# divideon/xvc

Hardware: AMD Instinct MI355X
Metric: hot-path frame passes/s (TZ + sub-pel ME, MC, transform + RDOQ + dequant + inverse, deblock, pad, PSNR parts), bit-exact vs the reference's classes (higher is better)
Workload: dtype u16; 1 GPU; 1920x1080 yuv420p 30fps synthetic, QP 32, internal bitdepth 10, 16x16 CUs, TZ range 96, RDOQ (RdoQuant::QuantRdo + CoeffSignHideRdo, picture-initial CABAC contexts); cus_per_picture=8160, parallelism=3 independent picture chains in flight

## Files before the change

### xvc_amd/csrc/k_quant.h

```cpp
#ifndef XVCGPU_K_QUANT_H_
#define XVCGPU_K_QUANT_H_

#include "dev_common.h"
#include "dev_tables.h"
#include "xvcgpu_internal.h"

struct TxBlockFlags {
  bool intra_pic;
  bool sign_hide;
  bool rdoq;
  int scan_order;
};
__device__ __forceinline__ TxBlockFlags tx_block_flags(int f) {
  return {(f & XVC_TXF_INTRA_PIC) != 0, !(f & XVC_TXF_NO_SIGN_HIDING), (f & XVC_TXF_RDOQ) != 0,
          (f >> XVC_TXF_SCAN_SHIFT) & 3};
}

__device__ __forceinline__ int rq_log2(int size) {
  return 31 - __clz(size);
}

struct BlockQuant {
  bool bias;
  int tshift;
  int scale;
  int shift;
  int size_bias_shift, size_bias_offset;
  int fq_shift;
  long long fq_offset;
  long long fast_offset;
  int iq_scale, iq_shift;
  int cost_scale;

  __device__ __forceinline__ int fwd(int a) const {
    return (int)(short)(int)((((long long)a * scale) + fq_offset) >> fq_shift);
  }
  __device__ __forceinline__ bool codes(int a) const { return fwd(a) != 0; }
  struct Fast {
    int16_t level, rem;
  };
  __device__ __forceinline__ Fast fast(int coeff) const {
    const int sign = coeff < 0 ? -1 : 1;
    const long long abs_coeff = d_abs(coeff);
    const int level = (int)(((abs_coeff * scale) + fast_offset) >> fq_shift);
    return {(int16_t)d_clip3(level * sign, -32768, 32767),
            (int16_t)(((abs_coeff * scale) - ((long long)level << fq_shift)) >> (fq_shift - 8))};
  }
  __device__ __forceinline__ int dequant(int level) const {
    const int prod = level * iq_scale;
    int cf;
    if (iq_shift > 0) cf = (prod + (1 << (iq_shift - 1))) >> iq_shift;
    else cf = (int)((unsigned)prod << -iq_shift);
    return (int)(short)d_clip3(cf, -32768, 32767);
  }
  __device__ __forceinline__ int err_of(int abs_coeff, int level) const {
    const long long orig_scaled =
        (((long long)abs_coeff * scale) + size_bias_offset) >> size_bias_shift;
    const long long quant_err = orig_scaled - ((long long)level << shift);
    return (int)(short)(quant_err >> (shift - 8));
  }
  __device__ __forceinline__ long long dist(int e) const {
    return ((long long)e * e) << cost_scale;
  }
  __device__ __forceinline__ long long zero_dist(int a) const {
    return ((long long)(a * a)) << cost_scale;
  }
};

__device__ __forceinline__ BlockQuant block_quant(int w, int h, int qp, int bd, bool intra_pic) {
  const int lsum = rq_log2(w) + rq_log2(h);
  int qpb = qp + 6 * (bd - 8);
  qpb = qpb > 0 ? qpb : 0;
  BlockQuant q;
  q.bias = (lsum & 1) != 0;
  q.tshift = 15 - bd - (lsum >> 1);
  q.scale = kFwdQuantScales[qpb % 6] * (q.bias ? 181 : 1);
  q.shift = 14 + qpb / 6 + q.tshift;
  q.size_bias_shift = q.bias ? 7 : 0;
  q.size_bias_offset = q.bias ? 64 : 0;
  q.fq_shift = q.shift + q.size_bias_shift;
  q.fq_offset = 1ll << (q.fq_shift - 1);
  q.fast_offset = (long long)((intra_pic ? 171ull : 85ull) << (q.fq_shift - 9));
  q.iq_scale = (kInvQuantScales[qpb % 6] << (qpb / 6)) * (q.bias ? 181 : 1);
  q.iq_shift = 6 - q.tshift + (q.bias ? 8 : 0);
  q.cost_scale = 15 - 2 * q.tshift - 2 * (bd - 8) + 2 * (q.bias ? 1 : 0);
  return q;
}
__device__ __forceinline__ BlockQuant block_quant(const xvcgpu_tx_block &b, int bd) {
  return block_quant(b.w, b.h, b.qp, bd, tx_block_flags(b.intra_pic).intra_pic);
}

struct TxStageShifts {
  int fwd1, fwd2, inv1, inv2;
  bool dct2_both;
};
__device__ __forceinline__ TxStageShifts tx_stage_shifts(int tx_hor, int tx_ver, int lgw, int lgh,
                                                         int bd) {
  const int hp_hor = tx_hor == XVC_TX_DCT2_LOW ? 0 : 2, hp_ver = tx_ver == XVC_TX_DCT2_LOW ? 0 : 2;
  auto dct2 = [](int t) { return t == XVC_TX_DEFAULT || t == XVC_TX_DCT2 || t == XVC_TX_DCT2_LOW; };
  return {lgw + bd - 9 + hp_hor, lgh + 6 + hp_ver, 7 + hp_ver, 20 - bd + hp_hor,
          dct2(tx_ver) && dct2(tx_hor)};
}
__device__ __forceinline__ TxStageShifts tx_stage_shifts_dst4(int bd) {
  TxStageShifts s = tx_stage_shifts(XVC_TX_DCT2_LOW, XVC_TX_DCT2_LOW, 2, 2, bd);
  s.dct2_both = false;
  return s;
}

__constant__ uint32_t kEntropyBits[128] = {
#include "entropy_bits.inc"
};
#define RQ_BYPASS 32768u
__device__ uint32_t gEntropyBits[128];

#define RQ_OFF(field) ((int)__builtin_offsetof(xvcgpu_rdoq_contexts, field))

__device__ __forceinline__ unsigned rq_bits(unsigned char state, int bin) {
  return kEntropyBits[state ^ bin];
}
__device__ __forceinline__ long long rq_bit_cost(unsigned bits, long long lambda) {
  return ((long long)bits * lambda) >> 16;
}

static_assert(sizeof(xvcgpu_rdoq_contexts) % 4 == 0, "whole words of contexts");
#define RQ_CTX_WORDS ((int)sizeof(xvcgpu_rdoq_contexts) / 4)
__device__ __forceinline__ void rq_stage_word(const uint32_t *table, uint32_t word, unsigned *cb8) {
#pragma unroll
  for (int k = 0; k < 4; k++) {
    const unsigned st8 = (word >> (8 * k)) & 127;
    *reinterpret_cast<uint2 *>(cb8 + 2 * k) = make_uint2(table[st8], table[st8 ^ 1]);
  }
}
__device__ __forceinline__ void rq_stage_costs(const uint32_t *table,
                                               const xvcgpu_rdoq_contexts *snap, unsigned *cb,
                                               int lane, int lanes) {
  const uint32_t *cw = reinterpret_cast<const uint32_t *>(snap);
  for (int wi = lane; wi < RQ_CTX_WORDS; wi += lanes) rq_stage_word(table, cw[wi], cb + 8 * wi);
}

__device__ __forceinline__ int rq_sig_ctx_base(bool luma, int posxy, int size_cls) {
  int start = posxy < 2 ? 6 : 0;
  start += luma && posxy < 5 ? 6 : 0;
  start += size_cls > 2 && luma ? 18 << (size_cls - 3 < 1 ? size_cls - 3 : 1) : 0;
  return 2 * ((luma ? RQ_OFF(sig_luma) : RQ_OFF(sig_chroma)) + start);
}
__device__ __forceinline__ int rq_greater1_off(bool luma) {
  return luma ? RQ_OFF(greater1_luma) : RQ_OFF(greater1_chroma);
}
__device__ __forceinline__ int rq_greater_start(bool luma, int posxy) {
  return luma ? (posxy < 3 ? 10 : (posxy < 10 ? 5 : 0)) : 0;
}
__device__ __forceinline__ int rq_greater_nn(int n, bool is_last) {
  return is_last ? 0 : (n < 4 ? n : 4) + 1;
}
__device__ __forceinline__ int rq_greater_ctx(bool luma, int posxy, int nn) {
  const int g1 = rq_greater1_off(luma);
  return nn == 0 ? 2 * g1 : 2 * (g1 + rq_greater_start(luma, posxy) + nn);
}

#endif
```

### xvc_amd/csrc/k_rdoq.h

```cpp
#ifndef XVCGPU_K_RDOQ_H_
#define XVCGPU_K_RDOQ_H_

#include "dev_common.h"
#include "k_me.h"
#include "k_me2.h"
#include "k_quant.h"
#include "k_rdoq4.h"
#include "k_rdoq_common.h"
#include "k_scan.h"
#include "xvcgpu_internal.h"


template <int G = 64, typename S, typename CF, typename LEV>
__device__ __forceinline__ int wave_rdoq(S &s, int lane, const BlockQuant &bq, int w, int h,
                                         bool luma, int scan_order, bool sign_hide,
                                         const xvcgpu_rdoq_contexts &ctx,
                                         const xvcgpu_rdoq_params &prm, CF cf, LEV lev,
                                         bool stage_ctx = true, bool clear_levels = true) {
  const int sbs = (w == 2 || h == 2) ? 1 : 2;
  const int sb_size = 1 << (2 * sbs);
  const int gw = w >> sbs, gh = h >> sbs;
  const int rw = w < 32 ? w : 32, rh = h < 32 ? h : 32;
  const int rgw = rw >> sbs, rgh = rh >> sbs;
  const int size_cls = (rq_log2(w) + rq_log2(h)) >> 1;
// ... 651 lines not shown
  l.part = base + 4 + 4 * (size_t)cap;
  return l;
}

__device__ __forceinline__ void rq_count_word(uint32_t v, int i, int end, int cnt[3]) {
#pragma unroll
  for (int k = 0; k < 4; k++) {
    const int c = (int)(signed char)(v >> (8 * k));
    const bool in = i + k < end;
    cnt[0] += in && c == 0;
    cnt[1] += in && c == 1;
    cnt[2] += in && c == 2;
  }
}
__device__ __forceinline__ int rq_wave_scan(int v) {
  const int lane = threadIdx.x & 63;
#pragma unroll
  for (int d = 1; d < 64; d <<= 1) {
    const int o = __shfl_up(v, d, 64);
    if (lane >= d) v += o;
  }
  return v;
}
template <int ROW>
__device__ __forceinline__ void rq_wave_totals_scan(int (&tot)[3][ROW]) {
  const int t = threadIdx.x;
  if (t < 64) {
#pragma unroll
    for (int k = 0; k < 3; k++) {
      int v = t < 16 ? tot[k][t] : 0;
#pragma unroll
      for (int d = 1; d < 16; d <<= 1) {
        const int o = __shfl_up(v, d, 64);
        if (t >= d) v += o;
      }
      if (t < 16) tot[k][16 + t] = v;
    }
  }
}
__device__ __forceinline__ void rq_scatter_word(uint32_t v, int i, int end, const RdoqLists &l,
                                                int pos[3]) {
#pragma unroll
  for (int k = 0; k < 4; k++) {
    const int c = (int)(signed char)(v >> (8 * k));
    if (i + k < end && c >= 0) l.list[c][pos[c]++] = i + k;
  }
}

__device__ __forceinline__ int rq_class_of(const xvcgpu_tx_block &b) {
  if (!rq4_takes(64, b.w, b.h, tx_block_flags(b.intra_pic).scan_order) || b.w > 32 || b.h > 32)
    return 2;
  const int n_sb = (b.w >> 2) * (b.h >> 2);
  return n_sb <= 4 ? 0 : (n_sb <= 16 ? 1 : 2);
}

__device__ __forceinline__ void rdoq_classify_kernel_body(int bd, const xvcgpu_tx_block *blocks, int n, const int16_t *coeffs, const uint32_t *d_off, int16_t *levels, int32_t *nnz_out, RdoqLists l) {
  const int bi = blockIdx.x * 4 + (int)(threadIdx.x >> 6);
  if (bi >= n) return;
  const int lane = threadIdx.x & 63;
  const xvcgpu_tx_block b = blocks[bi];
  const int w = b.w, h = b.h;
  const BlockQuant q = block_quant(b, bd);
  const int16_t *src = coeffs + d_off[bi];
  int16_t *dst = levels + d_off[bi];
  bool any = false;
  for (int i = lane; i < w * h; i += 64) any |= q.codes((short)d_abs((int)src[i]));
  if (__ballot(any)) {
    if (lane == 0) l.cls[bi] = (signed char)rq_class_of(b);
    return;
  }
  if (lane == 0) l.cls[bi] = -1;
  for (int i = lane; i < w * h; i += 64) dst[i] = 0;
  if (lane == 0 && nnz_out) nnz_out[bi] = 0;
}

__global__ void __launch_bounds__(256)
rdoq_classify_kernel(int bd, const xvcgpu_tx_block *blocks, int n, const int16_t *coeffs, const uint32_t *d_off, int16_t *levels, int32_t *nnz_out, RdoqLists l) {
  rdoq_classify_kernel_body(bd, blocks, n, coeffs, d_off, levels, nnz_out, l);
}

#define RQ_PROVE_BLOCKS 16
#define RQ_PROVE_MAX_CANDS 16

__device__ __forceinline__ int rq_prove_threshold(const BlockQuant &bq) {
  long long t = (long long)((double)bq.fq_offset / (double)bq.scale);
  while (t * bq.scale < bq.fq_offset) t++;
  while (t > 0 && (t - 1) * bq.scale >= bq.fq_offset) t--;
  return t > 32768 ? 32768 : (int)t;
}

template <class QAt>
__device__ __forceinline__ void rq_prove_candidate(const BlockQuant &bq, const xvcgpu_tx_block &b,
                                                   const xvcgpu_rdoq_params &prm,
                                                   const unsigned *cb, int x, int y, int a,
                                                   QAt qat, long long &gain, long long &gain_last,
                                                   long long &rhs, int &idx) {
  const int w = b.w, h = b.h, scan_order = tx_block_flags(b.intra_pic).scan_order;
  const bool luma = b.comp == 0;
  const long long lambda = prm.lambda;
  const int q = bq.fwd(a);
  int cnt, cnt1;
  {
    const int q0 = qat(x + 1, y), q1 = qat(x + 2, y), q2 = qat(x + 1, y + 1), q3 = qat(x, y + 1),
              q4 = qat(x, y + 2);
    cnt = (q0 > 0) + (q1 > 0) + (q2 > 0) + (q3 > 0) + (q4 > 0);
    cnt1 = (q0 > 1) + (q1 > 1) + (q2 > 1) + (q3 > 1) + (q4 > 1);
  }
  const int posxy = x + y;
  const int sig_base = rq_sig_ctx_base(luma, posxy, (rq_log2(w) + rq_log2(h)) >> 1);
  unsigned sig1 = 0xffffffffu;
  for (int nn = 0; nn <= cnt; nn++) {
    const unsigned v = cb[sig_base + 2 * nn + 1];
    sig1 = v < sig1 ? v : sig1;
  }
  const bool sub_dc = ((x | y) & 3) == 0 && (x | y) != 0;
  if (sub_dc) sig1 = 0;
  unsigned flag_min = RQ_BYPASS;
  auto meet = [&](int nn) {
    const int c = rq_greater_ctx(luma, posxy, nn);
    const unsigned v0 = cb[c], v1 = cb[c + 1];
    flag_min = v0 < flag_min ? v0 : flag_min;
    flag_min = v1 < flag_min ? v1 : flag_min;
  };
  meet(0);
  for (int n = 0; n <= cnt1; n++) meet(rq_greater_nn(n, false));
  const unsigned lvl_min = RQ_BYPASS + flag_min;
  long long d_best = bq.dist(a - bq.dequant(q));
  if (q > 1) {
    const long long d1 = bq.dist(a - bq.dequant(q - 1));
    d_best = d1 < d_best ? d1 : d_best;
  }
  const long long zd = bq.zero_dist(a);
  const long long coded = d_best + rq_bit_cost(sig1 + lvl_min, lambda);
  const long long coded_last = d_best + rq_bit_cost(lvl_min, lambda);
  gain = zd - (coded < zd ? coded : zd);
  gain_last = zd - coded_last;
  const unsigned lp = rq_last_pos_bits(cb, luma, w, h, scan_order, x, y);
  const int cbf_ctx = 2 * (!luma ? RQ_OFF(cbf_chroma)
                                 : ((prm.flags & XVC_RDOQ_INTRA_CU) ? RQ_OFF(cbf_luma)
                                                                    : RQ_OFF(root_cbf)));
  rhs = rq_bit_cost(cb[cbf_ctx + 1], lambda) - rq_bit_cost(cb[cbf_ctx], lambda) +
        rq_bit_cost(lp, lambda);
  constexpr unsigned long long inv0 = rq_pack_scan4_inv(0), inv1 = rq_pack_scan4_inv(1),
                               inv2 = rq_pack_scan4_inv(2);
  const unsigned long long inv = scan_order == 0 ? inv0 : (scan_order == 1 ? inv1 : inv2);
  const int kk = (int)((inv >> (4 * (((y & 3) << 2) | (x & 3)))) & 15ull);
  idx = (d_sb_scan_index(scan_order, w >> 2, h >> 2, x >> 2, y >> 2) << 4) + kk;
}

__global__ void __launch_bounds__(256)
rdoq_prove_zero_kernel(int bd, const xvcgpu_tx_block *blocks, int n, const int16_t *coeffs,
                       const uint32_t *d_off, int16_t *levels, int32_t *nnz_out,
                       const xvcgpu_rdoq_contexts *rq_ctx, const xvcgpu_rdoq_params *rq_prm,
                       RdoqLists l) {
  __shared__ __attribute__((aligned(16))) unsigned s_cb[2 * sizeof(xvcgpu_rdoq_contexts)];
  __shared__ unsigned short s_xy[16][RQ_PROVE_MAX_CANDS];
  __shared__ int s_idx[16][RQ_PROVE_MAX_CANDS];
  __shared__ long long s_gain[16][RQ_PROVE_MAX_CANDS];
  __shared__ int s_n[16];
  __shared__ int s_fail[16];
  __shared__ int s_ctx;
  const int g = threadIdx.x >> 4, gl = threadIdx.x & 15;
  const int base = blockIdx.x * RQ_PROVE_BLOCKS;
  if (threadIdx.x == 0) s_ctx = -1;
  __syncthreads();
  if ((int)threadIdx.x < RQ_PROVE_BLOCKS) {
    const int b2 = base + (int)threadIdx.x;
    if (b2 < n && l.cls[b2] >= 0) atomicMax(&s_ctx, (int)rq_prm[b2].ctx_index);
  }
  __syncthreads();
  const int wg_ctx = s_ctx;
  if (wg_ctx < 0) return;
  rq_stage_costs(gEntropyBits, &rq_ctx[wg_ctx], s_cb, (int)threadIdx.x, 256);
  __syncthreads();
  for (int sub = 0; sub < RQ_PROVE_BLOCKS / 16; sub++) {
    const int bi = base + sub * 16 + g;
    const bool live = bi < n && l.cls[bi < n ? bi : 0] >= 0;
    const xvcgpu_tx_block b = blocks[live ? bi : 0];
    const xvcgpu_rdoq_params prm = rq_prm[live ? bi : 0];
    if (gl == 0) {
      s_n[g] = 0;
      s_fail[g] = 0;
    }
    wave_sync();
    const BlockQuant bq = block_quant(b, bd);
    const int w = b.w, h = b.h;
    const int16_t *src = coeffs + d_off[live ? bi : 0];
    const bool tried = live && (int)prm.ctx_index == wg_ctx && w >= 4 && h >= 4 && w <= 32 &&
                       h <= 32 && (reinterpret_cast<uintptr_t>(src) & 7) == 0;
    auto qat = [&](int x, int y) {
      if (x >= w || y >= h) return 0;
      return bq.fwd((short)d_abs((int)src[y * w + x]));
    };
    if (tried) {
      const int thr = rq_prove_threshold(bq);
      bool wrap = false;
      for (int i = 4 * gl; i < w * h; i += 64) {
        const uint2 v = *reinterpret_cast<const uint2 *>(src + i);
        const int a4[4] = {d_abs((int)(short)(v.x & 0xffff)), d_abs((int)(short)(v.x >> 16)),
                           d_abs((int)(short)(v.y & 0xffff)), d_abs((int)(short)(v.y >> 16))};
#pragma unroll
        for (int t = 0; t < 4; t++) {
          wrap |= a4[t] == 32768;
          if (a4[t] >= thr) {
            const int slot = atomicAdd(&s_n[g], 1);
            const int ii = i + t;
            if (slot < RQ_PROVE_MAX_CANDS)
              s_xy[g][slot] = (unsigned short)(((ii >> rq_log2(w)) << 8) | (ii & (w - 1)));
          }
        }
      }
      if (wrap) s_fail[g] = 1;
    }
    wave_sync();
    const int nq = s_n[g];
    long long gain_last = 0, rhs = 0;
    int my_idx = 0;
    const bool cand = tried && nq <= RQ_PROVE_MAX_CANDS && gl < nq && !s_fail[g];
    if (tried && gl == 0 && (nq > RQ_PROVE_MAX_CANDS || nq == 0)) s_fail[g] = 1;
    if (cand) {
      const int x = s_xy[g][gl] & 255, y = s_xy[g][gl] >> 8;
      const int a = (short)d_abs((int)src[y * w + x]);
      long long gain;
      rq_prove_candidate(bq, b, prm, s_cb, x, y, a, qat, gain, gain_last, rhs, my_idx);
      s_idx[g][gl] = my_idx;
      s_gain[g][gl] = gain;
    }
    wave_sync();
    if (cand) {
      long long before = 0;
      for (int j = 0; j < nq; j++)
        if (s_idx[g][j] < my_idx) before += s_gain[g][j];
      if (before + gain_last >= rhs) s_fail[g] = 1;
    }
    wave_sync();
    if (tried && !s_fail[g]) {
      int16_t *dst = levels + d_off[bi];
      for (int i = gl; i < w * h; i += 16) dst[i] = 0;
      if (gl == 0) {
        if (nnz_out) nnz_out[bi] = 0;
        l.cls[bi] = -1;
      }
    }
    wave_sync();
  }
}

struct RqProveLds {
  __attribute__((aligned(16))) unsigned cb[2 * sizeof(xvcgpu_rdoq_contexts)];
  long long gain[2][RQ_PROVE_MAX_CANDS];
  int idx[2][RQ_PROVE_MAX_CANDS];
  unsigned short xy[2][RQ_PROVE_MAX_CANDS];
  int n[2];
  int fail[2];
  int staged_ctx;
};

template <int G>
__device__ __forceinline__ bool rq_prove_zero_lds(RqProveLds &pv, const xvcgpu_tx_block &b,
                                                  int bd,
                                                  const xvcgpu_rdoq_contexts *rq_ctx,
                                                  const xvcgpu_rdoq_params &prm,
                                                  const int16_t *c, bool live) {
  const int wl = (int)(threadIdx.x & 63), lane = wl & (G - 1), grp = wl / G;
  const int w = b.w, h = b.h;
  const int nq = pv.n[grp];
  bool tried = live && nq >= 1 && nq <= RQ_PROVE_MAX_CANDS && !pv.fail[grp] && w >= 4 && h >= 4 &&
               w <= 32 && h <= 32;
  const unsigned long long tm = __ballot(tried);
  if (!tm) return false;
  const int wave_ctx = __shfl((int)prm.ctx_index, __ffsll((long long)tm) - 1, 64);
  tried = tried && (int)prm.ctx_index == wave_ctx;
  if (pv.staged_ctx != wave_ctx) {
    wave_sync();
    rq_stage_costs(gEntropyBits, &rq_ctx[wave_ctx], pv.cb, wl, 64);
    if (wl == 0) pv.staged_ctx = wave_ctx;
    wave_sync();
  }
  const BlockQuant bq = block_quant(b, bd);
  auto qat = [&](int x, int y) {
    if (x >= w || y >= h) return 0;
    return bq.fwd((short)d_abs((int)c[x * h + y]));
  };
  long long gain_last = 0, rhs = 0;
  int my_idx = 0;
  const bool cand = tried && lane < nq;
  if (cand) {
    const int x = pv.xy[grp][lane] & 255, y = pv.xy[grp][lane] >> 8;
    const int a = (short)d_abs((int)c[x * h + y]);
    long long gain;
    rq_prove_candidate(bq, b, prm, pv.cb, x, y, a, qat, gain, gain_last, rhs, my_idx);
    pv.idx[grp][lane] = my_idx;
    pv.gain[grp][lane] = gain;
  }
  wave_sync();
  if (cand) {
    long long before = 0;
    for (int j = 0; j < nq; j++)
      if (pv.idx[grp][j] < my_idx) before += pv.gain[grp][j];
    if (before + gain_last >= rhs) pv.fail[grp] = 1;
  }
  wave_sync();
  return tried && !pv.fail[grp];
}

__device__ __forceinline__ void rdoq_compact_kernel_body(int n, RdoqLists l) {
  __shared__ int part[3][1024];
  const int t = threadIdx.x;
  const int per = ((n + 1023) / 1024 + 3) & ~3;
  const int a = t * per, e = a + per < n ? a + per : n;
  const uint32_t *cw = reinterpret_cast<const uint32_t *>(l.cls);
  int cnt[3] = {0, 0, 0};
  for (int i = a; i < e; i += 4) rq_count_word(cw[i >> 2], i, e, cnt);
#pragma unroll
  for (int k = 0; k < 3; k++) part[k][t] = cnt[k];
  __syncthreads();
  int inc[3];
#pragma unroll
  for (int k = 0; k < 3; k++) {
    inc[k] = rq_wave_scan(cnt[k]);
    if ((t & 63) == 63) part[k][t >> 6] = inc[k];
  }
  __syncthreads();
  rq_wave_totals_scan(part);
  __syncthreads();
  int pos[3];
#pragma unroll
  for (int k = 0; k < 3; k++)
    pos[k] = inc[k] - cnt[k] + ((t >> 6) ? part[k][16 + (t >> 6) - 1] : 0);
  for (int i = a; i < e; i += 4) rq_scatter_word(cw[i >> 2], i, e, l, pos);
  if (t == 1023)
    for (int k = 0; k < 3; k++) l.count[k] = part[k][16 + 15];
}

__global__ void __launch_bounds__(1024)
rdoq_count_kernel(int n, RdoqLists l) {
  __shared__ int wsum[3][16];
  const int t = threadIdx.x, i = (int)blockIdx.x * RDOQ_CHUNK + 4 * t;
  int cnt[3] = {0, 0, 0};
  if (i < n) rq_count_word(reinterpret_cast<const uint32_t *>(l.cls)[i >> 2], i, n, cnt);
#pragma unroll
  for (int k = 0; k < 3; k++) {
    const int v = wave_reduce_add_i32(cnt[k]);
    if ((t & 63) == 0) wsum[k][t >> 6] = v;
  }
  __syncthreads();
  if (t < 3) {
    int v = 0;
    for (int w = 0; w < 16; w++) v += wsum[t][w];
    l.part[4 * blockIdx.x + t] = v;
  }
}

__global__ void __launch_bounds__(1024)
rdoq_scatter_kernel(int n, RdoqLists l) {
  __shared__ int part[3][1024];
  __shared__ int base[3];
  const int t = threadIdx.x, b = blockIdx.x;
  {
    int v[3] = {0, 0, 0};
    for (int j = t; j < b; j += 1024) {
      v[0] += l.part[4 * j];
      v[1] += l.part[4 * j + 1];
      v[2] += l.part[4 * j + 2];
    }
#pragma unroll
    for (int k = 0; k < 3; k++) {
      const int w = wave_reduce_add_i32(v[k]);
      if ((t & 63) == 0) part[k][t >> 6] = w;
    }
    __syncthreads();
    if (t < 3) {
      int sum = 0;
      for (int w = 0; w < 16; w++) sum += part[t][w];
      base[t] = sum;
    }
    __syncthreads();
  }
  const int i = b * RDOQ_CHUNK + 4 * t;
  const uint32_t *cw = reinterpret_cast<const uint32_t *>(l.cls);
  int cnt[3] = {0, 0, 0};
  if (i < n) rq_count_word(cw[i >> 2], i, n, cnt);
  int inc[3];
#pragma unroll
  for (int k = 0; k < 3; k++) inc[k] = rq_wave_scan(cnt[k]);
  __syncthreads();
// ... 363 lines not shown
```

### xvc_amd/csrc/k_scan.h

```cpp
#ifndef XVCGPU_K_SCAN_H_
#define XVCGPU_K_SCAN_H_

#include "dev_common.h"

constexpr unsigned long long tx_pack_scan4(int order) {
  unsigned long long t = 0;
  int k = 0;
  if (order == 0) {
    for (int s = 0; s < 7; s++)
      for (int y = (s < 4 ? s : 3); y >= 0 && s - y < 4; y--, k++)
        t |= (unsigned long long)((y << 2) | (s - y)) << (4 * k);
  } else {
    for (k = 0; k < 16; k++)
      t |= (unsigned long long)(order == 1 ? k : (((k & 3) << 2) | (k >> 2))) << (4 * k);
  }
  return t;
}
__device__ __forceinline__ unsigned long long d_scan4_table(int order) {
  constexpr unsigned long long t0 = tx_pack_scan4(0), t1 = tx_pack_scan4(1),
                               t2 = tx_pack_scan4(2);
  return order == 0 ? t0 : (order == 1 ? t1 : t2);
}
__device__ __forceinline__ int d_sb_scan_index(int order, int gw, int gh, int sx, int sy) {
  if (order == 1) return sy * gw + sx;
  if (order == 2) return sx * gh + sy;
  const int s = sx + sy;
  int idx = 0;
  for (int d = 0; d < s; d++) {
    int c = d < gw - 1 ? d : gw - 1;
    c = c < gh - 1 ? c : gh - 1;
    c = c < gw + gh - 2 - d ? c : gw + gh - 2 - d;
    idx += c + 1;
  }
  return idx + ((s < gh - 1 ? s : gh - 1) - sy);
}

template <typename IDX>
__device__ __forceinline__ int d_sign_hide_subblock(int order, int px, int py,
                                                    bool is_last_sb, int16_t *lev,
                                                    const int16_t *dl, const int16_t *cf,
                                                    IDX idx) {
  const unsigned long long tab = d_scan4_table(order);
  auto at = [&](int k) {
    const int p = (int)((tab >> (4 * k)) & 15ull);
    return idx(px + (p & 3), py + (p >> 2));
  };
  int last = -1, first = 16, sum = 0;
  for (int k = 0; k < 16; k++) {
    const int c = lev[at(k)];
    if (c) {
      first = k < first ? k : first;
      last = k;
      sum += c;
    }
  }
  if (last - first <= 3) return 0;
  const int sign = lev[at(first)] > 0 ? 0 : 1;
  if (sign == (sum & 1)) return 0;
  int curr_cost = 32767, curr_change = 0, min_cost = 32767, min_change = 0, min_index = 0;
  for (int k = is_last_sb ? last : 15; k >= 0; k--) {
    const int p = at(k);
    const int l = lev[p], d = dl[p];
    if (l != 0) {
      if (d > 0) { curr_cost = -d; curr_change = 1; }
      else if (k == first && d_abs(l) == 1) curr_cost = 32767;
      else { curr_cost = d; curr_change = -1; }
    } else if (k < first && (cf[p] >= 0 ? 0 : 1) != sign) {
      curr_cost = 32767;
    } else {
      curr_cost = -d;
      curr_change = 1;
    }
    if (curr_cost < min_cost) { min_cost = curr_cost; min_change = curr_change; min_index = k; }
  }
  const int p = at(min_index);
  const int before = lev[p];
  if (before == -32768 || before == 32767) min_change = -1;
  const int after = (int16_t)(before + (cf[p] >= 0 ? min_change : -min_change));
  lev[p] = (int16_t)after;
  return (after != 0) - (before != 0);
}

constexpr unsigned long long rq_pack_scan4_inv(int order) {
  const unsigned long long t = tx_pack_scan4(order);
  unsigned long long r = 0;
  for (int k = 0; k < 16; k++) r |= (unsigned long long)k << (4 * (int)((t >> (4 * k)) & 15ull));
  return r;
}

#endif
```

### xvc_amd/csrc/k_tx2.h

```cpp
#ifndef XVCGPU_K_TX2_H_
#define XVCGPU_K_TX2_H_

#include "dev_common.h"
#include "dev_tables.h"
#include "k_me.h"
#include "k_me2.h"
#include "k_quant.h"
#include "k_rdoq.h"
#include "k_tx.h"
#include "xvcgpu_internal.h"

#define TX2_WAVES 4

typedef short tx2_v2s __attribute__((ext_vector_type(2)));

struct __attribute__((aligned(16))) Tx2Shared {
  int16_t r[256];
  int16_t t[256];
  int16_t c[256];
};

__device__ __forceinline__ int tx2_dot2(uint32_t a, uint32_t b, int acc) {
  return __builtin_amdgcn_sdot2(__builtin_bit_cast(tx2_v2s, a),
                                __builtin_bit_cast(tx2_v2s, b), acc, false);
// ... 79 lines not shown
  signed char *cls;
  int16_t *levels;
  int32_t *nnz;
  const xvcgpu_rdoq_contexts *rq_ctx;
  const xvcgpu_rdoq_params *rq_prm;
  RqProveLds *pv;
};

template <int MODE, int G = 64, bool RDOQ = false, int FW = 0, int FH = 0>
__device__ __forceinline__ int tx2_job(Tx2Shared &sh, const xvcgpu_tx_block &b, int bi,
                                       int bd, const PlaneView &po, const uint16_t *pred_p,
                                       int pred_stride, const PlaneView &pr,
                                       int16_t *levels, const uint32_t *level_off,
                                       int32_t *nnz_out, const int16_t *tx_tables,
                                       const int16_t *tx_tables_t,
                                       const TxTableLayout &lay,
                                       const U16x4 *orig_pre = nullptr, int soff = 0,
                                       RdoqShared<(G == 32 ? 64 : 256)> *rq = nullptr,
                                       const xvcgpu_rdoq_contexts *rq_ctx = nullptr,
                                       const xvcgpu_rdoq_params *rq_prm = nullptr,
                                       unsigned long long *dist_out = nullptr,
                                       const FwdClassify *fc = nullptr) {
  struct { int16_t *r, *t, *c; } s = {sh.r + soff, sh.t + soff, sh.c + soff};
  unsigned long long dist_acc = 0;
  auto dist4 = [&](int y, int x, const U16x4 &p, int r0, int r1, int r2, int r3) {
    const U16x4 o = *reinterpret_cast<const U16x4 *>(po.p + (ptrdiff_t)(b.y + y) * po.stride +
                                                     b.x + x);
    const int d0 = (int)(o.v[0] & 0xffff) - (int)(p.v[0] & 0xffff) - r0;
    const int d1 = (int)(o.v[0] >> 16) - (int)(p.v[0] >> 16) - r1;
    const int d2 = (int)(o.v[1] & 0xffff) - (int)(p.v[1] & 0xffff) - r2;
    const int d3 = (int)(o.v[1] >> 16) - (int)(p.v[1] >> 16) - r3;
    dist_acc += (unsigned long long)((long long)d0 * d0) + (unsigned long long)((long long)d1 * d1) +
                (unsigned long long)((long long)d2 * d2) + (unsigned long long)((long long)d3 * d3);
  };
  auto dist_finish = [&]() {
    unsigned long long v = dist_acc;
#pragma unroll
    for (int sft = 1; sft < G; sft <<= 1) v += __shfl_xor(v, sft, 64);
    if ((ME2_LANE & (G - 1)) == 0) dist_out[bi] = v >> (2 * (bd - 8));
  };
  const int lane = ME2_LANE & (G - 1);
  const int w = FW ? FW : b.w, h = FH ? FH : b.h;
  const int lw = 31 - __clz(w);
  const int lgw = lw, lgh = 31 - __clz(h);
  int16_t *lv = (levels && level_off) ? levels + level_off[bi] : nullptr;
  const int offh = tx_table_off(lay, b.tx_hor, w), offv = tx_table_off(lay, b.tx_ver, h);
  const int16_t *Mh = tx_tables + offh, *Mv = tx_tables + offv;
  const int16_t *MhT = tx_tables_t + offh, *MvT = tx_tables_t + offv;

  const TxBlockFlags fl = tx_block_flags(b.intra_pic);
  auto quant = [&]() { return block_quant(w, h, b.qp, bd, fl.intra_pic); };
  const int n_el = w * h;
  constexpr int NE = FW * FH;

  int nnz;
  if (MODE != TX_MODE_INV) {
    lane_loop<NE, 4 * G>(lane * 4, n_el, [&](int i) {
      const int y = i >> lw, x = i & (w - 1);
      const U16x4 o = orig_pre ? *orig_pre
                               : *reinterpret_cast<const U16x4 *>(
                                     po.p + (ptrdiff_t)(b.y + y) * po.stride + b.x + x);
      const U16x4 p = *reinterpret_cast<const U16x4 *>(
          pred_p + (ptrdiff_t)y * pred_stride + x);
      const int d0 = (int)(o.v[0] & 0xffff) - (int)(p.v[0] & 0xffff);
      const int d1 = (int)(o.v[0] >> 16) - (int)(p.v[0] >> 16);
      const int d2 = (int)(o.v[1] & 0xffff) - (int)(p.v[1] & 0xffff);
      const int d3 = (int)(o.v[1] >> 16) - (int)(p.v[1] >> 16);
      *reinterpret_cast<uint2 *>(s.r + i) =
          make_uint2((uint32_t)(d0 & 0xffff) | ((uint32_t)d1 << 16),
                     (uint32_t)(d2 & 0xffff) | ((uint32_t)d3 << 16));
    });
    wave_sync();
    ME2_TRACE(2);
    const TxStageShifts st = tx_stage_shifts(b.tx_hor, b.tx_ver, lgw, lgh, bd);
    tx2_stage_dispatch<false, G>(w, Mh, s.r, w, h, 1 << (st.fwd1 - 1), st.fwd1, s.t);
    wave_sync();
    ME2_TRACE(3);
    tx2_stage_dispatch<false, G>(h, s.t, Mv, w, h, 1 << (st.fwd2 - 1), st.fwd2, s.c);
    wave_sync();
    ME2_TRACE(4);
    if (MODE == TX_MODE_FWD) {
      if (fc && fc->cls) {
        const BlockQuant q = quant();
        bool any = false;
        RqProveLds *pv = fc->pv;
        const int grp = ME2_LANE / G;
        if (pv) {
          if (lane == 0) {
            pv->n[grp] = 0;
            pv->fail[grp] = 0;
          }
          wave_sync();
        }
        lane_loop<NE, G>(lane, n_el, [&](int i) {
          const int a = (short)d_abs((int)s.c[i]);
          const bool nz = q.codes(a);
          any |= nz;
          if (pv && nz) {
            const int slot = atomicAdd(&pv->n[grp], 1);
            if (slot < RQ_PROVE_MAX_CANDS)
              pv->xy[grp][slot] = (unsigned short)(((i & (h - 1)) << 8) | (i >> lgh));
            if (a < 0) pv->fail[grp] = 1;
          }
        });
        const unsigned long long group =
            G == 64 ? ~0ull : (((1ull << G) - 1) << (ME2_LANE & ~(G - 1)));
        bool live = (__ballot(any) & group) != 0;
        if (pv) {
          wave_sync();
          if (rq_prove_zero_lds<G>(*pv, b, bd, fc->rq_ctx, fc->rq_prm[bi], s.c, live)) live = false;
        }
        if (lane == 0) fc->cls[bi] = live ? (signed char)rq_class_of(b) : (signed char)-1;
        if (!live) {
          int16_t *z = fc->levels + level_off[bi];
          lane_loop<NE, G>(lane, n_el, [&](int i) { z[i] = 0; });
          if (lane == 0 && fc->nnz) fc->nnz[bi] = 0;
          return 0;
        }
      }
      if (lv)
        lane_loop<NE, G>(lane, n_el, [&](int i) {
          const int x = i >> lgh, k2 = i & (h - 1);
          lv[k2 * w + x] = s.c[i];
        });
      return 0;
    }
    const bool sign_hide = fl.sign_hide;
    const int scan_order = fl.scan_order;
    const bool use_rdoq = RDOQ && fl.rdoq;
    const BlockQuant q = quant();
    if (RDOQ && use_rdoq) {
      const xvcgpu_rdoq_params prm = rq_prm[bi];
      const int16_t *cfp = s.c;
      int16_t *lvp = s.r;
      auto cf_at = [cfp, h](int x, int y) { return (int)cfp[x * h + y]; };
      auto lv_at = [lvp, h](int x, int y) { return lvp + x * h + y; };
      if (G == 64 && rq4_takes(64, w, h, scan_order)) {
        rq_stage_costs(kEntropyBits, &rq_ctx[prm.ctx_index], rq->ctx_bits, lane, 64);
        wave_sync();
        nnz = wave_rdoq4<64, 1>(*rq, lane, q, w, h, b.comp == 0, sign_hide, prm, cf_at, lv_at);
      } else {
        nnz = wave_rdoq<G>(*rq, lane, q, w, h, b.comp == 0, scan_order, sign_hide,
                           rq_ctx[prm.ctx_index], prm, cf_at, lv_at);
      }
      wave_sync();
    }
    int local = 0;
    if (!use_rdoq) {
    for (int i = lane; i < n_el; i += G) {
      const BlockQuant::Fast f = q.fast(s.c[i]);
      local += f.level != 0;
      s.r[i] = f.level;
      s.t[i] = f.rem;
    }
    nnz = tx2_group_add<G>(local);
    }
    if (!use_rdoq && sign_hide && nnz > 1 && w >= 4 && h >= 4) {
      wave_sync();
      const int gw = w >> 2, gh = h >> 2;
      auto idx = [h](int x, int y) { return x * h + y; };
      const bool mine = lane < gw * gh;
      const int sx = mine ? (lane & (gw - 1)) : 0, sy = mine ? (lane >> (lgw - 2)) : 0;
      bool any = false;
      if (mine)
        for (int k = 0; k < 16; k++) any |= s.r[idx(4 * sx + (k & 3), 4 * sy + (k >> 2))] != 0;
      const int my_scan = d_sb_scan_index(scan_order, gw, gh, sx, sy);
      int last_sb = any ? my_scan : -1;
#pragma unroll
      for (int sft = 1; sft < 16; sft <<= 1) {
        const int o = __shfl_xor(last_sb, sft, 64);
        last_sb = o > last_sb ? o : last_sb;
      }
      int dn = 0;
      if (mine)
        dn = d_sign_hide_subblock(scan_order, 4 * sx, 4 * sy, my_scan == last_sb, s.r, s.t,
                                  s.c, idx);
      nnz += tx2_group_add<G>(dn);
    }
    if (nnz_out && lane == 0) nnz_out[bi] = nnz;
    if (lv) {
      wave_sync();
      for (int i = lane; i < n_el; i += G) {
        const int x = i >> lgh, k2 = i & (h - 1);
        lv[k2 * w + x] = s.r[i];
      }
    }
  } else {
    nnz = nnz_out[bi];
    if (nnz)
      lane_loop<NE, G>(lane, n_el, [&](int i) {
        const int x = i >> lgh, k2 = i & (h - 1);
        s.r[i] = lv[k2 * w + x];
      });
  }
  wave_sync();

  if (nnz == 0) {
    if (MODE == TX_MODE_INV && !dist_out &&
// ... 217 lines not shown
```

Before: 9074 frame passes/s.

## Rework RDOQ zero-proof: threshold tables, ballot compaction, DPP cost rows

The forward classification pass now tests each coefficient against a precomputed per-scale/shift magnitude threshold instead of multiplying by the quant scale. Candidates are compacted with ballot/mbcnt instead of LDS atomics, which drops the counter and fail-flag LDS state and several wave syncs. For 8x8 and 16x16 blocks, the proof builds its context-cost rows with DPP prefix sums and cross-lane shuffles rather than staging the full cost table in LDS. The before-sum is read with vector loads and all-zero blocks are cleared with 16-byte stores. The added table and specialized paths carry a bit-exactness risk at edge cases, such as a magnitude of 32768 or a lambda that exceeds 32 bits.

```diff
diff --git a/xvc_amd/csrc/k_quant.h b/xvc_amd/csrc/k_quant.h
--- a/xvc_amd/csrc/k_quant.h
+++ b/xvc_amd/csrc/k_quant.h
@@ -24,6 +24,7 @@
   bool bias;
   int tshift;
   int scale;
+  int scale_idx;
   int shift;
   int size_bias_shift, size_bias_offset;
   int fq_shift;
@@ -75,6 +76,7 @@
   q.bias = (lsum & 1) != 0;
   q.tshift = 15 - bd - (lsum >> 1);
   q.scale = kFwdQuantScales[qpb % 6] * (q.bias ? 181 : 1);
+  q.scale_idx = qpb % 6 + (q.bias ? 6 : 0);
   q.shift = 14 + qpb / 6 + q.tshift;
   q.size_bias_shift = q.bias ? 7 : 0;
   q.size_bias_offset = q.bias ? 64 : 0;
@@ -88,6 +90,41 @@
 }
 __device__ __forceinline__ BlockQuant block_quant(const xvcgpu_tx_block &b, int bd) {
   return block_quant(b.w, b.h, b.qp, bd, tx_block_flags(b.intra_pic).intra_pic);
+}
+
+#define RQ_THR_SHIFTS 48
+struct RqLevelThrTable {
+  unsigned short t[12][RQ_THR_SHIFTS][2];
+};
+constexpr RqLevelThrTable rq_make_level_thr_table() {
+  constexpr int fwd[6] = {26214, 23302, 20560, 18396, 16384, 14564};
+  RqLevelThrTable r{};
+  for (int i = 0; i < 12; i++) {
+    const unsigned long long scale = (unsigned long long)(fwd[i % 6] * (i < 6 ? 1 : 181));
+    for (int s = 0; s < RQ_THR_SHIFTS; s++) {
+      for (int m = 0; m < 2; m++) {
+        unsigned long long t = 65535;
+        if (s >= 1) {
+          const unsigned long long target = (m ? 3ull : 1ull) << (s - 1);
+          t = (target + scale - 1) / scale;
+          if (m == 0 && t == 32768 && t * scale == target) t = 32769;
+          if (t > 65535) t = 65535;
+        }
+        r.t[i][s][m] = (unsigned short)t;
+      }
+    }
+  }
+  return r;
+}
+__constant__ RqLevelThrTable kRqLevelThr = rq_make_level_thr_table();
+struct RqLevelThr {
+  int t1, t2;
+};
+__device__ __forceinline__ RqLevelThr rq_level_thresholds(const BlockQuant &bq) {
+  if (bq.fq_shift < 0 || bq.fq_shift >= RQ_THR_SHIFTS) return {65535, 65535};
+  const uint32_t v =
+      *reinterpret_cast<const uint32_t *>(kRqLevelThr.t[bq.scale_idx][bq.fq_shift]);
+  return {(int)(v & 0xffff), (int)(v >> 16)};
 }
 
 struct TxStageShifts {
diff --git a/xvc_amd/csrc/k_rdoq.h b/xvc_amd/csrc/k_rdoq.h
--- a/xvc_amd/csrc/k_rdoq.h
+++ b/xvc_amd/csrc/k_rdoq.h
@@ -757,6 +757,53 @@
 #define RQ_PROVE_BLOCKS 16
 #define RQ_PROVE_MAX_CANDS 16
 
+template <bool NARROW>
+__device__ __forceinline__ void rq_prove_price(const BlockQuant &bq, long long lambda, int a,
+                                               unsigned sig1, unsigned flag_min, unsigned lp,
+                                               unsigned cbf0, unsigned cbf1, long long &gain,
+                                               long long &gain_last, long long &rhs) {
+  auto price = [&](unsigned bits) -> long long {
+    if (NARROW)
+      return (long long)(((unsigned long long)bits * (unsigned long long)(unsigned)lambda) >> 16);
+    return rq_bit_cost(bits, lambda);
+  };
+  auto dist = [&](int e) -> long long {
+    return (long long)((unsigned long long)((unsigned)e * (unsigned)e)) << bq.cost_scale;
+  };
+  const int q = bq.fwd(a);
+  const unsigned lvl_min = RQ_BYPASS + flag_min;
+  long long d_best = dist(a - bq.dequant(q));
+  if (q > 1) {
+    const long long d1 = dist(a - bq.dequant(q - 1));
+    d_best = d1 < d_best ? d1 : d_best;
+  }
+  const long long zd = bq.zero_dist(a);
+  const long long coded = d_best + price(sig1 + lvl_min);
+  const long long coded_last = d_best + price(lvl_min);
+  gain = zd - (coded < zd ? coded : zd);
+  gain_last = zd - coded_last;
+  rhs = price(cbf1) - price(cbf0) + price(lp);
+}
+
+template <int W, int H>
+__device__ __forceinline__ int rq_prove_scan_index(int scan_order, int w, int h, int x, int y) {
+  constexpr unsigned long long inv0 = rq_pack_scan4_inv(0), inv1 = rq_pack_scan4_inv(1),
+                               inv2 = rq_pack_scan4_inv(2);
+  const unsigned long long inv = scan_order == 0 ? inv0 : (scan_order == 1 ? inv1 : inv2);
+  const int kk = (int)((inv >> (4 * (((y & 3) << 2) | (x & 3)))) & 15ull);
+  int sb;
+  if constexpr (W >= 4 && H >= 4 && (W >> 2) * (H >> 2) <= 16) {
+    constexpr int GW = W >> 2, GH = H >> 2;
+    constexpr unsigned long long kSb = rq_pack_sb_scan(GW, GH);
+    const int sx = x >> 2, sy = y >> 2;
+    sb = scan_order == 0 ? (int)((kSb >> (4 * (sy * GW + sx))) & 15ull)
+                         : (scan_order == 1 ? sy * GW + sx : sx * GH + sy);
+  } else {
+    sb = d_sb_scan_index(scan_order, w >> 2, h >> 2, x >> 2, y >> 2);
+  }
+  return (sb << 4) + kk;
+}
+
 __device__ __forceinline__ int rq_prove_threshold(const BlockQuant &bq) {
   long long t = (long long)((double)bq.fq_offset / (double)bq.scale);
   while (t * bq.scale < bq.fq_offset) t++;
@@ -923,60 +970,168 @@
 
 struct RqProveLds {
   __attribute__((aligned(16))) unsigned cb[2 * sizeof(xvcgpu_rdoq_contexts)];
-  long long gain[2][RQ_PROVE_MAX_CANDS];
-  int idx[2][RQ_PROVE_MAX_CANDS];
+  __attribute__((aligned(16))) long long gain[2][RQ_PROVE_MAX_CANDS];
+  __attribute__((aligned(16))) int idx[2][RQ_PROVE_MAX_CANDS];
   unsigned short xy[2][RQ_PROVE_MAX_CANDS];
-  int n[2];
-  int fail[2];
   int staged_ctx;
 };
 
 template <int G>
+__device__ __forceinline__ void rq_prove_collect(RqProveLds *pv, bool hit, int i, int h, int lgh,
+                                                 int &nq) {
+  static_assert(G == 64 || G == 32, "a wave or half a wave per block");
+  const unsigned long long hits = __ballot(hit);
+  if (!hits) return;
+  const unsigned lo = (unsigned)hits, hi = (unsigned)(hits >> 32);
+  int below, total;
+  if (G == 64) {
+    below = (int)__builtin_amdgcn_mbcnt_hi(hi, __builtin_amdgcn_mbcnt_lo(lo, 0u));
+    total = __popc(lo) + __popc(hi);
+  } else {
+    const bool up = (threadIdx.x & 32) != 0;
+    below = up ? (int)__builtin_amdgcn_mbcnt_hi(hi, 0u) : (int)__builtin_amdgcn_mbcnt_lo(lo, 0u);
+    total = up ? __popc(hi) : __popc(lo);
+  }
+  const int slot = nq + below;
+  if (pv && hit && slot < RQ_PROVE_MAX_CANDS)
+    pv->xy[(threadIdx.x & 63) / G][slot] = (unsigned short)(((i & (h - 1)) << 8) | (i >> lgh));
+  nq += total;
+}
+
+struct RqProveRow {
+  unsigned t, zero, one;
+};
+template <int S>
+__device__ __forceinline__ RqProveRow rq_prove_tables(const xvcgpu_rdoq_contexts *snap, bool luma,
+                                                      bool intra_cu) {
+  static_assert(S == 16 || S == 8, "last-position groups 0 .. 7 fit a row");
+  constexpr int LS = S == 16 ? 4 : 3;
+  const int wl = (int)(threadIdx.x & 63), t = wl & 7, row = wl >> 3;
+  const int gmax = rq_last_pos_group(S - 1), gc = gmax - 1;
+  const int tc = t < 5 ? t : 5;
+  int ctx;
+  if (row < 2) {
+    ctx = rq_last_pos_ctx(luma, S, S, t < gc ? t : gc, row == 0) >> 1;
+  } else if (row < 5) {
+    ctx = (rq_sig_ctx_base(luma, row == 2 ? 0 : (row == 3 ? 2 : 5), LS) >> 1) + tc;
+    if (wl == 22)
+      ctx = !luma ? RQ_OFF(cbf_chroma) : (intra_cu ? RQ_OFF(cbf_luma) : RQ_OFF(root_cbf));
+  } else {
+    const int g1 = rq_greater1_off(luma);
+    ctx = t == 0 ? g1 : g1 + rq_greater_start(luma, row == 5 ? 0 : (row == 6 ? 3 : 10)) + tc;
+  }
+  const unsigned st = reinterpret_cast<const unsigned char *>(snap)[ctx] & 127u;
+  const unsigned zero = gEntropyBits[st], one = gEntropyBits[st ^ 1u];
+  const bool sum = row < 2;
+  const unsigned own = row < 5 ? one : (zero < one ? zero : one);
+  unsigned v = own;
+  auto step = [&](unsigned got, int s) {
+    if (t >= s) v = sum ? v + got : (got < v ? got : v);
+  };
+  step((unsigned)__builtin_amdgcn_update_dpp(0, (int)v, 0x111, 0xF, 0xF, false), 1);
+  step((unsigned)__builtin_amdgcn_update_dpp(0, (int)v, 0x112, 0xF, 0xF, false), 2);
+  step((unsigned)__builtin_amdgcn_update_dpp(0, (int)v, 0x114, 0xF, 0xF, false), 4);
+  unsigned tv;
+  if (sum)
+    tv = v - own + (t < gmax ? zero : 0u) + (t > 3 ? (unsigned)((t - 2) >> 1) * RQ_BYPASS : 0u);
+  else if (row < 5)
+    tv = v;
+  else
+    tv = v < RQ_BYPASS ? v : RQ_BYPASS;
+  return {tv, zero, one};
+}
+
+template <int G, int W, int H>
 __device__ __forceinline__ bool rq_prove_zero_lds(RqProveLds &pv, const xvcgpu_tx_block &b,
-                                                  int bd,
+                                                  int w, int h, const BlockQuant &bq,
+                                                  const RqLevelThr &thr,
                                                   const xvcgpu_rdoq_contexts *rq_ctx,
-                                                  const xvcgpu_rdoq_params &prm,
-                                                  const int16_t *c, bool live) {
+                                                  const xvcgpu_rdoq_params *rq_prm, int bi,
+                                                  const int16_t *c, int nq) {
   const int wl = (int)(threadIdx.x & 63), lane = wl & (G - 1), grp = wl / G;
-  const int w = b.w, h = b.h;
-  const int nq = pv.n[grp];
-  bool tried = live && nq >= 1 && nq <= RQ_PROVE_MAX_CANDS && !pv.fail[grp] && w >= 4 && h >= 4 &&
-               w <= 32 && h <= 32;
+  const unsigned long long group = G == 64 ? ~0ull : (((1ull << G) - 1) << (wl & ~(G - 1)));
+  bool tried = nq >= 1 && nq <= RQ_PROVE_MAX_CANDS && w >= 4 && h >= 4 && w <= 32 && h <= 32;
   const unsigned long long tm = __ballot(tried);
   if (!tm) return false;
+  const xvcgpu_rdoq_params prm = rq_prm[bi];
   const int wave_ctx = __shfl((int)prm.ctx_index, __ffsll((long long)tm) - 1, 64);
   tried = tried && (int)prm.ctx_index == wave_ctx;
-  if (pv.staged_ctx != wave_ctx) {
-    wave_sync();
-    rq_stage_costs(gEntropyBits, &rq_ctx[wave_ctx], pv.cb, wl, 64);
-    if (wl == 0) pv.staged_ctx = wave_ctx;
-    wave_sync();
-  }
-  const BlockQuant bq = block_quant(b, bd);
-  auto qat = [&](int x, int y) {
-    if (x >= w || y >= h) return 0;
-    return bq.fwd((short)d_abs((int)c[x * h + y]));
-  };
-  long long gain_last = 0, rhs = 0;
-  int my_idx = 0;
+  wave_sync();
+  long long gain = 0, gain_last = 0, rhs = 0;
+  int my_idx = 0x7fffffff;
+  bool over = false;
   const bool cand = tried && lane < nq;
-  if (cand) {
-    const int x = pv.xy[grp][lane] & 255, y = pv.xy[grp][lane] >> 8;
-    const int a = (short)d_abs((int)c[x * h + y]);
-    long long gain;
-    rq_prove_candidate(bq, b, prm, pv.cb, x, y, a, qat, gain, gain_last, rhs, my_idx);
+  if constexpr (W == H && (W == 16 || W == 8)) {
+    auto mag = [&](int x, int y) {
+      if (x >= W || y >= H) return 0;
+      return d_abs((int)c[x * H + y]);
+    };
+    const bool narrow = __ballot(cand && (unsigned long long)prm.lambda > 0xffffffffull) == 0;
+    const int scan_order = tx_block_flags(b.intra_pic).scan_order;
+    const bool luma = __builtin_amdgcn_readfirstlane((int)(b.comp == 0)) != 0;
+    const RqProveRow row =
+        rq_prove_tables<W>(&rq_ctx[wave_ctx], luma, (prm.flags & XVC_RDOQ_INTRA_CU) != 0);
+    const unsigned xy = cand ? pv.xy[grp][lane] : 0u;
+    const int x = (int)(xy & 255u), y = (int)(xy >> 8);
+    const int a = d_abs((int)c[x * H + y]);
+    over = a == 32768;
+    const int m0 = mag(x + 1, y), m1 = mag(x + 2, y), m2 = mag(x + 1, y + 1), m3 = mag(x, y + 1),
+              m4 = mag(x, y + 2);
+    const int cnt =
+        (m0 >= thr.t1) + (m1 >= thr.t1) + (m2 >= thr.t1) + (m3 >= thr.t1) + (m4 >= thr.t1);
+    const int cnt1 =
+        (m0 >= thr.t2) + (m1 >= thr.t2) + (m2 >= thr.t2) + (m3 >= thr.t2) + (m4 >= thr.t2);
+    const int posxy = x + y;
+    const int scls = (posxy >= 2) + (posxy >= 5), gcls = (posxy >= 3) + (posxy >= 10);
+    unsigned sig1 = __shfl(row.t, 16 + 8 * scls + cnt, 64);
+    const unsigned flag_min = __shfl(row.t, 40 + 8 * gcls + rq_greater_nn(cnt1, false), 64);
+    const unsigned lp = __shfl(row.t, rq_last_pos_group(scan_order == 2 ? y : x), 64) +
+                        __shfl(row.t, 8 + rq_last_pos_group(scan_order == 2 ? x : y), 64);
+    const unsigned cbf0 = __shfl(row.zero, 22, 64), cbf1 = __shfl(row.one, 22, 64);
+    if (((x | y) & 3) == 0 && (x | y) != 0) sig1 = 0;
+    if (narrow)
+      rq_prove_price<true>(bq, prm.lambda, a, sig1, flag_min, lp, cbf0, cbf1, gain, gain_last, rhs);
+    else
+      rq_prove_price<false>(bq, prm.lambda, a, sig1, flag_min, lp, cbf0, cbf1, gain, gain_last,
+                            rhs);
+    if (cand) my_idx = rq_prove_scan_index<W, H>(scan_order, W, H, x, y);
+  } else {
+    if (pv.staged_ctx != wave_ctx) {
+      rq_stage_costs(gEntropyBits, &rq_ctx[wave_ctx], pv.cb, wl, 64);
+      if (wl == 0) pv.staged_ctx = wave_ctx;
+      wave_sync();
+    }
+    auto qat = [&](int x, int y) {
+      if (x >= w || y >= h) return 0;
+      return bq.fwd((short)d_abs((int)c[x * h + y]));
+    };
+    if (cand) {
+      const int x = pv.xy[grp][lane] & 255, y = pv.xy[grp][lane] >> 8;
+      const int a = d_abs((int)c[x * h + y]);
+      over = a == 32768;
+      rq_prove_candidate(bq, b, prm, pv.cb, x, y, a, qat, gain, gain_last, rhs, my_idx);
+    }
+  }
+  if (tried && lane < RQ_PROVE_MAX_CANDS) {
     pv.idx[grp][lane] = my_idx;
     pv.gain[grp][lane] = gain;
   }
   wave_sync();
+  bool bad = false;
   if (cand) {
     long long before = 0;
-    for (int j = 0; j < nq; j++)
-      if (pv.idx[grp][j] < my_idx) before += pv.gain[grp][j];
-    if (before + gain_last >= rhs) pv.fail[grp] = 1;
-  }
-  wave_sync();
-  return tried && !pv.fail[grp];
+    for (int j = 0; j < nq; j += 4) {
+      const int4 id = *reinterpret_cast<const int4 *>(&pv.idx[grp][j]);
+      const longlong2 g01 = *reinterpret_cast<const longlong2 *>(&pv.gain[grp][j]);
+      const longlong2 g23 = *reinterpret_cast<const longlong2 *>(&pv.gain[grp][j + 2]);
+      before += id.x < my_idx ? g01.x : 0ll;
+      before += id.y < my_idx ? g01.y : 0ll;
+      before += id.z < my_idx ? g23.x : 0ll;
+      before += id.w < my_idx ? g23.y : 0ll;
+    }
+    bad = over || before + gain_last >= rhs;
+  }
+  return tried && (__ballot(bad) & group) == 0;
 }
 
 __device__ __forceinline__ void rdoq_compact_kernel_body(int n, RdoqLists l) {
diff --git a/xvc_amd/csrc/k_scan.h b/xvc_amd/csrc/k_scan.h
--- a/xvc_amd/csrc/k_scan.h
+++ b/xvc_amd/csrc/k_scan.h
@@ -21,7 +21,7 @@
                                t2 = tx_pack_scan4(2);
   return order == 0 ? t0 : (order == 1 ? t1 : t2);
 }
-__device__ __forceinline__ int d_sb_scan_index(int order, int gw, int gh, int sx, int sy) {
+__attribute__((always_inline)) constexpr int sb_scan_index(int order, int gw, int gh, int sx, int sy) {
   if (order == 1) return sy * gw + sx;
   if (order == 2) return sx * gh + sy;
   const int s = sx + sy;
@@ -33,6 +33,16 @@
     idx += c + 1;
   }
   return idx + ((s < gh - 1 ? s : gh - 1) - sy);
+}
+__device__ __forceinline__ int d_sb_scan_index(int order, int gw, int gh, int sx, int sy) {
+  return sb_scan_index(order, gw, gh, sx, sy);
+}
+constexpr unsigned long long rq_pack_sb_scan(int gw, int gh) {
+  unsigned long long r = 0;
+  for (int sy = 0; sy < gh; sy++)
+    for (int sx = 0; sx < gw; sx++)
+      r |= (unsigned long long)sb_scan_index(0, gw, gh, sx, sy) << (4 * (sy * gw + sx));
+  return r;
 }
 
 template <typename IDX>
diff --git a/xvc_amd/csrc/k_tx2.h b/xvc_amd/csrc/k_tx2.h
--- a/xvc_amd/csrc/k_tx2.h
+++ b/xvc_amd/csrc/k_tx2.h
@@ -185,38 +185,45 @@
     if (MODE == TX_MODE_FWD) {
       if (fc && fc->cls) {
         const BlockQuant q = quant();
-        bool any = false;
+        const RqLevelThr thr = rq_level_thresholds(q);
         RqProveLds *pv = fc->pv;
-        const int grp = ME2_LANE / G;
-        if (pv) {
-          if (lane == 0) {
-            pv->n[grp] = 0;
-            pv->fail[grp] = 0;
+        int nq = 0;
+        auto look = [&](int i, int cf) {
+          rq_prove_collect<G>(pv, i < n_el && d_abs(cf) >= thr.t1, i, h, lgh, nq);
+        };
+        if constexpr (NE > 0) {
+          constexpr int PER = NE / G;
+          static_assert(PER * G == NE && (PER == 2 || PER == 4), "16x16 by a wave, 8x8 by half");
+          if constexpr (PER == 4) {
+            const uint2 v = *reinterpret_cast<const uint2 *>(s.c + 4 * lane);
+            look(4 * lane, (int)(short)(v.x & 0xffff));
+            look(4 * lane + 1, (int)v.x >> 16);
+            look(4 * lane + 2, (int)(short)(v.y & 0xffff));
+            look(4 * lane + 3, (int)v.y >> 16);
+          } else {
+            const uint32_t v = *reinterpret_cast<const uint32_t *>(s.c + 2 * lane);
+            look(2 * lane, (int)(short)(v & 0xffff));
+            look(2 * lane + 1, (int)v >> 16);
           }
-          wave_sync();
+        } else {
+          for (int i0 = 0; i0 < n_el; i0 += G) {
+            const int i = i0 + lane;
+            look(i, i < n_el ? (int)s.c[i] : 0);
+          }
         }
-        lane_loop<NE, G>(lane, n_el, [&](int i) {
-          const int a = (short)d_abs((int)s.c[i]);
-          const bool nz = q.codes(a);
-          any |= nz;
-          if (pv && nz) {
-            const int slot = atomicAdd(&pv->n[grp], 1);
-            if (slot < RQ_PROVE_MAX_CANDS)
-              pv->xy[grp][slot] = (unsigned short)(((i & (h - 1)) << 8) | (i >> lgh));
-            if (a < 0) pv->fail[grp] = 1;
-          }
-        });
-        const unsigned long long group =
-            G == 64 ? ~0ull : (((1ull << G) - 1) << (ME2_LANE & ~(G - 1)));
-        bool live = (__ballot(any) & group) != 0;
-        if (pv) {
-          wave_sync();
-          if (rq_prove_zero_lds<G>(*pv, b, bd, fc->rq_ctx, fc->rq_prm[bi], s.c, live)) live = false;
-        }
+        bool live = nq != 0;
+        if (pv && rq_prove_zero_lds<G, FW, FH>(*pv, b, w, h, q, thr, fc->rq_ctx, fc->rq_prm, bi,
+                                               s.c, nq))
+          live = false;
         if (lane == 0) fc->cls[bi] = live ? (signed char)rq_class_of(b) : (signed char)-1;
         if (!live) {
           int16_t *z = fc->levels + level_off[bi];
-          lane_loop<NE, G>(lane, n_el, [&](int i) { z[i] = 0; });
+          if ((n_el & 7) == 0 && (reinterpret_cast<uintptr_t>(z) & 15) == 0)
+            lane_loop<NE, 8 * G>(lane * 8, n_el, [&](int i) {
+              *reinterpret_cast<uint4 *>(z + i) = make_uint4(0u, 0u, 0u, 0u);
+            });
+          else
+            lane_loop<NE, G>(lane, n_el, [&](int i) { z[i] = 0; });
           if (lane == 0 && fc->nnz) fc->nnz[bi] = 0;
           return 0;
         }
```

Result: faster. 9289 frame passes/s, median of 6 (+2.4%).
